# patrick-bedkowski/Generative-DNN-for-Physics-Simulations-CERN

Hardware: AMD Instinct MI355X
Metric: GAN-step images/sec (44x44 ZDC) at 1/2/4/8 MI355X; conv MFMA util % (higher is better)
Workload: dtype fp32

## Files before the change

### generative-dnn-for-physics-simulations-cern_amd/csrc/conv_common.h

```cpp
#pragma once
#include "common.h"

enum { MODE_FWD = 0, MODE_DGRAD = 1, MODE_WGRAD = 2 };

struct FastDiv {
  uint32_t m;
  int l;
};
static inline FastDiv mkdiv(uint32_t d) {
  FastDiv f;
  f.l = 0;
  while ((1ull << f.l) < d) ++f.l;
  f.m = (uint32_t)(((1ull << 32) * ((1ull << f.l) - d)) / d + 1);
  return f;
}
__device__ __forceinline__ int fdiv(int x, FastDiv f) {
  return (int)((__umulhi((uint32_t)x, f.m) + (uint32_t)x) >> f.l);
}

struct SubPixel {
  int on;
  int ph[4], pw[4];
  int p0[4], q0[4];
  int oh[4], ow[4];
// ... 56 lines not shown
}

__device__ __forceinline__ void conv_live_gemm(ConvArgs& a, int mode) {
  a.mslot = a.M;
  if (a.d.rows == nullptr) return;
  const int nl = conv_live(a), npx = conv_live_px(a);
  if (mode == MODE_WGRAD) a.Kd = min(nl * (a.Kd / a.d.N), npx);
  else a.M = min(nl * (a.M / a.d.N), npx);
}


struct DetRequest {
  float* ws;
  int64_t floats;
  int splits;
};
extern thread_local DetRequest g_det_req;

struct BnRedRequest {
  const void* x;
  const es_norm_t* nm;
  const es_chain_t* ch;
  float* part;
  int64_t floats;
  int chunks;
};
extern thread_local BnRedRequest g_bnr_req;



struct StatsRequest {
  float* part;
  int64_t floats;
  int chunks;
};
extern thread_local StatsRequest g_stats_req;

struct AffineRequest {
  const float* scale;
  const float* shift;
  int act;
  float slope;
  int fused;
};
extern thread_local AffineRequest g_aff_req;
int es_f32_split_level();

extern thread_local int g_ring_hit;

extern "C" int64_t es_weight_planes_offset(int64_t n);

int es_conv_ring_launch(ConvArgs& a, int mode, hipStream_t st);
int es_conv_ring_launch_f32(ConvArgs& a, int mode, hipStream_t st);
int64_t es_wgrad_f32_ring_floats(const es_conv_desc_t& d, const int64_t ys[4], const int64_t xs[4]);
int es_wgrad_f32_ring(const es_conv_desc_t& d, const void* dy, const int64_t ys[4], const void* x,
                      const int64_t xs[4], float* dw, float beta, float* ws, int64_t ws_floats, hipStream_t st);
int es_wgrad_ws_launch(int bn, bool sp, dim3 grid, const ConvArgs& a, float* wsc, int ngt, hipStream_t st);
void es_wgrad_reduce_plain(const float* ws, int splits, int K, int C, int R, int S, float* dw, float beta,
                           hipStream_t st);
```

### generative-dnn-for-physics-simulations-cern_amd/csrc/conv_mfma.hip

```cpp
#include <algorithm>
#include <cstdio>
#include <cstdlib>
#include <type_traits>

#include "conv_common.h"
#include "ring_common.h"
#include "split_fp32.h"


namespace {

constexpr int RT = 512;
constexpr int NSLOT = 3;
constexpr int SPB_PFD = 2;
constexpr int SPB_DMA_HI = 6;

bool g_ring_off = false;
int g_wgrad_ws = 1;

template <typename F>
struct lambda_arg : lambda_arg<decltype(&F::operator())> {};
template <typename C, typename R, typename A0, typename... As>
struct lambda_arg<R (C::*)(A0, As...) const> {
  typedef A0 type;
};


struct ClsReg {
  uint64_t v;
  __device__ __forceinline__ void init(const int* src) {
    uint32_t lo = ((uint32_t)(uint16_t)src[0]) | ((uint32_t)(uint16_t)src[1] << 16);
    uint32_t hi = ((uint32_t)(uint16_t)src[2]) | ((uint32_t)(uint16_t)src[3] << 16);
    v = ((uint64_t)(uint32_t)uni((int)hi) << 32) | (uint32_t)uni((int)lo);
  }
  __device__ __forceinline__ int operator()(int c) const { return (int)(short)(uint16_t)(v >> (16 * c)); }
};

template <int BK = 64>
__device__ __forceinline__ int swz_x(int row) {
  return BK == 64 ? ((row >> 1) & 7) : ((0x78 >> (2 * ((row >> 2) & 3))) & 3);
}
template <int BK = 64>
__device__ __forceinline__ int swz(int row, int chunk) { return row * (BK * 2) + ((chunk ^ swz_x<BK>(row)) << 4); }

typedef short short4_t __attribute__((ext_vector_type(4)));
typedef short short8_t __attribute__((ext_vector_type(8)));

template <int BROWS>
__device__ __forceinline__ int swz_tr(int k) {
  if constexpr (BROWS >= 128) return ((k & 3) << 1) | (((k >> 3) & 1) << 3);
  else return (((k >> 1) & 1) << 1) | (((k >> 3) & 1) << 2);
}

template <int BROWS>
__device__ __forceinline__ int tr_off(int k, int row) {
  return k * (BROWS * 2) + ((((row >> 3) ^ swz_tr<BROWS>(k)) << 4) | ((row & 7) << 1));
}

template <int BROWS>
__device__ __forceinline__ bf16x8 tr_frag(const char* img, int k0, int r0) {
  const int lane = threadIdx.x & 63;
  const int g = lane >> 4, q = (lane >> 2) & 3, p = lane & 3;
  const int ka = k0 + 8 * g + q;
  const char* p0 = img + tr_off<BROWS>(ka, r0 + 4 * p);
  const char* p1 = img + tr_off<BROWS>(ka + 4, r0 + 4 * p);
  short4_t lo = __builtin_amdgcn_ds_read_tr16_b64_v4i16((__attribute__((address_space(3))) short4_t*)p0);
  short4_t hi = __builtin_amdgcn_ds_read_tr16_b64_v4i16((__attribute__((address_space(3))) short4_t*)p1);
  short8_t v = {lo[0], lo[1], lo[2], lo[3], hi[0], hi[1], hi[2], hi[3]};
  return __builtin_bit_cast(bf16x8, v);
}

typedef int int2v __attribute__((ext_vector_type(2)));
typedef int int4v __attribute__((ext_vector_type(4)));
typedef unsigned int v4u32_t __attribute__((ext_vector_type(4)));
__device__ __forceinline__ uint32_t lds_u32(const void* p) {
  return (uint32_t)(uintptr_t)(const __attribute__((address_space(3))) void*)p;
}
__device__ __forceinline__ int2v ds_tr16(uint32_t addr) {
  int2v r;
  asm volatile("ds_read_b64_tr_b16 %0, %1" : "=v"(r) : "v"(addr));
  return r;
}
template <int BROWS>
__device__ __forceinline__ bf16x8 tr_frag_asm(uint32_t img, int k0, int r0) {
  const int lane = threadIdx.x & 63;
  const int g = lane >> 4, q = (lane >> 2) & 3, p = lane & 3;
  const int ka = k0 + 8 * g + q;
  const int2v lo = ds_tr16(img + tr_off<BROWS>(ka, r0 + 4 * p));
  const int2v hi = ds_tr16(img + tr_off<BROWS>(ka + 4, r0 + 4 * p));
  const int4v v = {lo[0], lo[1], hi[0], hi[1]};
  return __builtin_bit_cast(bf16x8, v);
}
__device__ __forceinline__ void fence_frag(bf16x8& x) {
  int4v v = __builtin_bit_cast(int4v, x);
  asm volatile("" : "+v"(v));
  x = __builtin_bit_cast(bf16x8, v);
// ... 2264 lines not shown
        for (int z = q; z < splits; z += WR_LANES, p += WR_LANES * zst) {
#pragma unroll
          for (int cl = 0; cl < 4; ++cl) {
            const float4 w = *(const float4*)(p + off[cl]);
            v.x += w.x; v.y += w.y; v.z += w.z; v.w += w.w;
          }
        }
      } else {
        const int off = (r * S + s) * C;
#pragma unroll 4
        for (int z = q; z < splits; z += WR_LANES, p += WR_LANES * zst) {
          const float4 w = *(const float4*)(p + off);
          v.x += w.x; v.y += w.y; v.z += w.z; v.w += w.w;
        }
      }
    }
    part[q][o] = v;
    __syncthreads();
    if (q == 0 && i < n4) {
      float4 u = part[0][o];
#pragma unroll
      for (int l = 1; l < WR_LANES; ++l) {
        const float4 w = part[l][o];
        u.x += w.x; u.y += w.y; u.z += w.z; u.w += w.w;
      }
      const float uu[4] = {u.x, u.y, u.z, u.w};
#pragma unroll
      for (int j = 0; j < 4; ++j) {
        float* g = dw + (((int64_t)k * C + c + j) * R + r) * S + s;
        *g = (beta != 0.f ? beta * *g : 0.f) + uu[j];
      }
    }
    __syncthreads();
  }
}

static void launch_wgrad_reduce(const float* ws, int splits, int K, int C, int R, int S, int ngt, const SubPixel& sp,
                                float* dw, float beta, hipStream_t st) {
  if (C % 4 == 0 && ngt % 4 == 0) {
    const int64_t n4 = (int64_t)K * C / 4 * R * S;
    const int blocks = (int)std::min<int64_t>((n4 + 31) / 32, 16384);
    hipLaunchKernelGGL(wgrad_reduce4_kernel, dim3(blocks), dim3(256), 0, st, ws, splits, K, C, R, S, ngt, sp, dw, beta);
    return;
  }
  const int64_t n = (int64_t)K * C * R * S;
  const int blocks = (int)std::min<int64_t>((n + 31) / 32, 16384);
  hipLaunchKernelGGL(wgrad_reduce_kernel, dim3(blocks), dim3(256), 0, st, ws, splits, K, C, R, S, ngt, sp, dw, beta);
}
int64_t g_conv_launches = 0;
extern "C" int64_t es_conv_launch_count() { return g_conv_launches; }

template <int MODE, int BM, int BN, bool SP, int BK, typename T, int SPL>
void launch_ring_grid(const ConvArgs& a, dim3 grid, hipStream_t st, bool aff) {
  if constexpr (MODE == MODE_FWD && (sizeof(T) == 2 || SPL > 0)) {
    if (aff) {
      g_aff_req.fused = 1;
      hipLaunchKernelGGL((conv_ring_kernel<MODE, BM, BN, SP, BK, T, SPL, true>), grid, dim3(RT), 0, st, a);
      return;
    }
  }
  hipLaunchKernelGGL((conv_ring_kernel<MODE, BM, BN, SP, BK, T, SPL>), grid, dim3(RT), 0, st, a);
}

template <int MODE, int BM, int BN, bool SP, int BK = 64, typename T = bf16, int SPL = 0>
void launch_ring(const ConvArgs& a, int row_tiles, hipStream_t st, bool aff = false) {
  dim3 grid(row_tiles, (a.Ng + BN - 1) / BN, 1);
  ++g_conv_launches;
  launch_ring_grid<MODE, BM, BN, SP, BK, T, SPL>(a, grid, st, aff);
}

constexpr int WGRAD_MINK = 8;
template <int BM, int BN, bool SP>
void launch_wgrad_ring(ConvArgs& a, hipStream_t st) {
  const int taps = SP ? a.sp.tap0[4] : a.d.R * a.d.S;
  const int tiles = (a.M / BM) * (taps * a.d.C / BN);
  int npix = a.d.P * a.d.Q;
  if (SP)
    for (int c = 0; c < 4; ++c) npix = c == 0 ? a.sp.ph[0] * a.sp.pw[0] : max(npix, a.sp.ph[c] * a.sp.pw[c]);
  const int ks = npix * ((a.d.N + 63) / 64);
  const int want = max(1, min(ks / WGRAD_MINK, 512 / tiles));
  const int per = (ks + want - 1) / want;
  a.k_per_split = per;
  dim3 grid(a.M / BM, taps * a.d.C / BN, (ks + per - 1) / per);
  ++g_conv_launches;
  hipLaunchKernelGGL((wgrad_ring_kernel<BM, BN, SP>), grid, dim3(RT), 0, st, a);
}

template <int EB>
bool dense_small_t(const int64_t s[4], int n, int c, int h, int w) {
  return s[1] == 1 && s[3] == c && s[2] == (int64_t)w * c && s[0] == (int64_t)h * w * c &&
         (int64_t)n * s[0] * EB < (1ll << 30);
}
bool dense_small(const int64_t s[4], int n, int c, int h, int w) { return dense_small_t<2>(s, n, c, h, w); }

constexpr int RING_NG = 64;
constexpr int RING_NG_DYN = 16;
bool g_subpixel_off = false;
bool g_ring256 = true;
bool g_persist = true;
bool g_p256 = true;

}

thread_local StatsRequest g_stats_req;
thread_local AffineRequest g_aff_req;
thread_local BnRedRequest g_bnr_req;

void es_make_subpixel(const es_conv_desc_t& d, int row_tile, SubPixel& sp) {
  int dhv[2], dwv[2], p0v[2], q0v[2], phv[2], pwv[2], ohv[2], owv[2];
  for (int a = 0; a < 2; ++a) {
    dhv[a] = ((a + d.R - 1) >> 1) + 1;
    dwv[a] = ((a + d.S - 1) >> 1) + 1;
    p0v[a] = (a + d.pad) & 1;
    q0v[a] = (a + d.pad) & 1;
    phv[a] = d.P > p0v[a] ? (d.P - p0v[a] + 1) / 2 : 0;
    pwv[a] = d.Q > q0v[a] ? (d.Q - q0v[a] + 1) / 2 : 0;
    ohv[a] = (p0v[a] - d.pad - a) / 2;
    owv[a] = (q0v[a] - d.pad - a) / 2;
  }
  sp.on = 1;
  sp.tap0[0] = 0;
  sp.tile0[0] = 0;
  for (int c = 0; c < 4; ++c) {
    const int a = c >> 1, b = c & 1;
    sp.ph[c] = phv[a];
    sp.pw[c] = pwv[b];
    sp.p0[c] = p0v[a];
    sp.q0[c] = q0v[b];
    sp.oh[c] = ohv[a];
    sp.ow[c] = owv[b];
    sp.dh[c] = dhv[a];
    sp.dw[c] = dwv[b];
    sp.tap0[c + 1] = sp.tap0[c] + dhv[a] * dwv[b];
    const int pix = phv[a] * pwv[b];
    sp.tile0[c + 1] = sp.tile0[c] + (row_tile > 0 ? (pix + row_tile - 1) / row_tile : 0);
  }
}

extern "C" int es_conv_set_ring(int on) {
  const int old = !g_ring_off;
  g_ring_off = !on;
  return old;
}

extern "C" int es_conv_set_persist(int on) {
  const int old = g_persist ? 1 : 0;
  g_persist = (on & 1) != 0;
  return old;
}

extern "C" int es_conv_set_p256(int on) {
  const int old = g_p256;
  g_p256 = on != 0;
  return old;
}

extern "C" int es_conv_set_ring256(int on) {
  const int old = g_ring256;
  g_ring256 = on != 0;
  return old;
}

extern "C" int es_conv_set_subpixel(int on) {
  const int old = !g_subpixel_off;
  g_subpixel_off = !on;
  return old;
}

extern "C" int es_subpixel_taps(int R, int S) {
  return (((R - 1) >> 1) + 1 + (R >> 1) + 1) * (((S - 1) >> 1) + 1 + (S >> 1) + 1);
}

extern "C" int es_conv_subpixel_ok(const es_conv_desc_t* d, es_dtype_t dt) {
  if (g_ring_off || g_subpixel_off || !d || (dt != ES_BF16 && dt != ES_F32)) return 0;
  if (d->up_h != 2 || d->up_w != 2 || d->hmap || d->stride != 1) return 0;
  if (d->C % 64 || d->K % 64) return 0;
  const int eb = dt == ES_F32 ? 4 : 2;
  const int64_t xbytes = (int64_t)d->N * d->H * d->W * d->C * eb, ybytes = (int64_t)d->N * d->P * d->Q * d->K * eb;
  const int64_t wbytes = (int64_t)d->K * d->C * es_subpixel_taps(d->R, d->S) * eb;
  if (dt == ES_F32) return wbytes < (1ll << 30) && (int64_t)d->H * d->W * d->C * eb < (1ll << 24) &&
                           (int64_t)d->P * d->Q * d->K * eb < (1ll << 24);
  (void)xbytes; (void)ybytes;
  return wbytes < (1ll << 30) && (int64_t)d->H * d->W * d->C * eb < (1ll << 24) &&
         (int64_t)d->P * d->Q * d->K * eb < (1ll << 24);
}

template <typename T, int SPL = 0>
int ring_fd(ConvArgs& a, int mode, hipStream_t st);
namespace {
int chunk_images(int64_t img_bytes, int N);
int ring_launch_chunks(ConvArgs& a, int mode, int nc, hipStream_t st);
}

int es_conv_ring_launch(ConvArgs& a, int mode, hipStream_t st) {
  const es_conv_desc_t& d = a.d;
  const bool sp_weights = d.subpixel != 0;
// ... 460 lines not shown
```

### generative-dnn-for-physics-simulations-cern_amd/csrc/ring_common.h

```cpp
#pragma once
#include "common.h"

namespace {

constexpr uint32_t OOB = 0x80000000u;

typedef __attribute__((address_space(3))) void lds_void;

__device__ __forceinline__ __amdgpu_buffer_rsrc_t mkres(const void* p, uint32_t bytes) {
  return __builtin_amdgcn_make_buffer_rsrc((void*)p, (short)0, (int)bytes, 0x00020000);
}
__device__ __forceinline__ void bdma16(__amdgpu_buffer_rsrc_t r, uint32_t voff, char* lds_wave_base) {
  __builtin_amdgcn_raw_ptr_buffer_load_lds(r, (lds_void*)lds_wave_base, 16, (int)voff, 0, 0, 0);
}

__device__ __forceinline__ void ring_barrier() { asm volatile("s_barrier" ::: "memory"); }

template <int N>
__device__ __forceinline__ void wait_vmcnt() {
  asm volatile("s_waitcnt vmcnt(%0)" ::"n"(N) : "memory");
}

__device__ __forceinline__ int xcd_remap(int orig, int nwg) {
  const int q8 = nwg / 8, r8 = nwg % 8, xcd = orig % 8;
  return (xcd < r8 ? xcd * (q8 + 1) : r8 * (q8 + 1) + (xcd - r8) * q8) + orig / 8;
}

__device__ __forceinline__ int uni(int v) { return __builtin_amdgcn_readfirstlane(v); }

}
```

### generative-dnn-for-physics-simulations-cern_amd/expertsim/hip.py

```python
from __future__ import annotations

import ctypes as C
import os

import numpy as np
import torch

_LIB_PATH = os.environ.get("ES_LIB") or os.path.join(os.path.dirname(os.path.abspath(__file__)), "_lib",
                                                     "libexpertsim_hip.so")
_lib = None

ES_F32, ES_BF16 = 0, 1
ACT_NONE, ACT_RELU, ACT_LRELU = 0, 1, 2
NORM_NONE, NORM_BN, NORM_GN, NORM_LN = 0, 1, 2, 3


class View(C.Structure):
    _fields_ = [("n", C.c_int), ("c", C.c_int), ("h", C.c_int), ("w", C.c_int), ("s", C.c_int64 * 4),
                ("rows", C.c_void_p)]


class Dropout(C.Structure):
    _fields_ = [("seed", C.c_uint64), ("stream", C.c_uint32), ("threshold", C.c_uint32),
                ("scale", C.c_float), ("enabled", C.c_int), ("step_ptr", C.c_void_p), ("step_mul", C.c_int32),
# ... 27 lines not shown
class DFront2Params(C.Structure):
    _fields_ = [("w1", C.c_void_p), ("sigma1", C.c_void_p), ("b1", C.c_void_p), ("g1", C.c_void_p),
                ("be1", C.c_void_p), ("w2", C.c_void_p), ("sigma2", C.c_void_p), ("b2", C.c_void_p),
                ("g2", C.c_void_p), ("be2", C.c_void_p), ("eps1", C.c_float), ("eps2", C.c_float),
                ("slope", C.c_float), ("ph", C.c_int), ("pw", C.c_int), ("rows", C.c_void_p)]


class DMlpParams(C.Structure):
    _fields_ = [("w1", C.c_void_p), ("sigma1", C.c_void_p), ("b1", C.c_void_p), ("g1", C.c_void_p),
                ("be1", C.c_void_p), ("w2", C.c_void_p), ("sigma2", C.c_void_p), ("b2", C.c_void_p),
                ("g2", C.c_void_p), ("be2", C.c_void_p), ("w3", C.c_void_p), ("sigma3", C.c_void_p),
                ("b3", C.c_void_p), ("eps1", C.c_float), ("eps2", C.c_float), ("slope", C.c_float),
                ("rows", C.c_void_p)]


class PackJob(C.Structure):
    _fields_ = [("w", C.c_void_p), ("K", C.c_int), ("C", C.c_int), ("R", C.c_int), ("S", C.c_int),
                ("mode", C.c_int), ("dt", C.c_int), ("planes", C.c_int), ("out", C.c_void_p)]


class Affine(C.Structure):
    _fields_ = [("scale", C.c_void_p), ("shift", C.c_void_p), ("act", C.c_int), ("slope", C.c_float)]


P = C.c_void_p
I64 = C.c_int64
_SIGS = {
    "es_last_error": (C.c_char_p, []),
    "es_version": (C.c_int, []),
    "es_device_sync": (C.c_int, []),
    "es_conv_set_glds": (C.c_int, [C.c_int]),
    "es_conv_set_ring": (C.c_int, [C.c_int]),
    "es_conv_set_subpixel": (C.c_int, [C.c_int]),
    "es_conv_set_ring256": (C.c_int, [C.c_int]),
    "es_conv_set_persist": (C.c_int, [C.c_int]),
    "es_conv_set_p256": (C.c_int, [C.c_int]),
    "es_conv_subpixel_ok": (C.c_int, [P, C.c_int]),
    "es_subpixel_taps": (C.c_int, [C.c_int, C.c_int]),
    "es_conv2d_fwd": (C.c_int, [P, C.c_int, P, P, P, P, P, C.c_int, P, P]),
    "es_conv2d_fwd_stats": (C.c_int, [P, C.c_int, P, P, P, P, P, C.c_int, P, P, I64, P, P]),
    "es_conv2d_fwd_affine": (C.c_int, [P, C.c_int, P, P, P, P, P, P, C.c_int, P, P, P]),
    "es_conv2d_dgrad": (C.c_int, [P, C.c_int, P, P, P, P, C.c_int, P, C.c_float, P]),
    "es_conv2d_dgrad_bnred": (C.c_int, [P, C.c_int, P, P, P, P, C.c_int, P, P, P, P, P, I64, P, P]),
    "es_conv2d_wgrad": (C.c_int, [P, C.c_int, P, P, P, P, P, P]),
    "es_conv2d_wgrad_det_ws_bytes": (I64, [P, C.c_int, P, P]),
    "es_conv2d_wgrad_det": (C.c_int, [P, C.c_int, P, P, P, P, P, C.c_float, P, I64, P]),
    "es_set_deterministic": (C.c_int, [C.c_int]),
    "es_conv2d_splitk_ws_bytes": (I64, [P, C.c_int]),
    "es_conv2d_fwd_det": (C.c_int, [P, C.c_int, P, P, P, P, P, C.c_int, P, P, I64, P]),
    "es_conv2d_dgrad_det": (C.c_int, [P, C.c_int, P, P, P, P, C.c_int, P, P, I64, P]),
    "es_conv_set_f32_chunk": (C.c_int, [C.c_int]),
    "es_conv_set_f32_split": (C.c_int, [C.c_int]),
    "es_conv_set_wgrad_ws": (C.c_int, [C.c_int]),
    "es_weight_planes_offset": (C.c_int64, [C.c_int64]),
    "es_pack_weight_planes": (C.c_int, [P, C.c_int64, P, P]),
    "es_pack_conv_weights": (C.c_int, [P, C.c_int, P]),
    "es_conv_launch_count": (C.c_int64, []),
    "es_conv_exec_flops": (C.c_int, [C.POINTER(C.c_double), C.c_int]),
    "es_pack_conv_weight": (C.c_int, [P, C.c_int, C.c_int, C.c_int, C.c_int, C.c_int, P, P, P, C.c_int, P]),
    "es_unpack_conv_grad": (C.c_int, [P, C.c_int, C.c_int, C.c_int, C.c_int, P, P, C.c_float, P]),
    "es_unpack_conv_grad_clear": (C.c_int, [P, C.c_int, C.c_int, C.c_int, C.c_int, P, C.c_float, P]),
    "es_norm_stats_ws_bytes": (I64, [P, C.c_int, C.c_int]),
    "es_norm_stats": (C.c_int, [P, C.c_int, P, C.c_int, C.c_int, C.c_float, P, P, P, P, C.c_float, P, P]),
    "es_norm_act_fwd": (C.c_int, [P, C.c_int, P, P, P, C.c_int, P, P, P, C.c_int, P, P]),
    "es_norm_stats_finalize": (C.c_int, [P, C.c_int, C.c_int, C.c_float, P, P, P, P, C.c_float, P]),
    "es_norm_bwd_ws_bytes": (I64, [P, C.c_int, C.c_int]),
    "es_norm_act_bwd": (C.c_int, [P, C.c_int, P, P, P, P, C.c_int, P, P, C.c_int, P, P, C.c_int, P,
                                  C.c_float, P, P, P, P, P]),
    "es_norm_act_bwd_sums": (C.c_int, [P, C.c_int, P, P, P, P, C.c_int, P, P, C.c_int, P, P, C.c_int, P, P, P,
                                       P, P]),
    "es_norm_stats_merge": (C.c_int, [P, C.c_int, C.c_int, P, P]),
    "es_norm_stats_local": (C.c_int, [P, C.c_int, P, P, P, P]),
    "es_norm_bwd_sync": (C.c_int, [C.c_int, P, C.c_int, P, P, P, P, C.c_int, P, P, C.c_int, P, P, C.c_float, P, P,
                                   P, P, P, P]),
    "es_act_fwd": (C.c_int, [P, C.c_int, P, P, P, C.c_int, P, P]),
    "es_dropout_keep_bits": (C.c_int, [P, P, P]),
    "es_channel_sum_ws_bytes": (I64, [P]),
    "es_channel_sum": (C.c_int, [P, C.c_int, P, P, C.c_float, P, P]),
    "es_maxpool_fwd": (C.c_int, [P, C.c_int, P, C.c_int, C.c_int, C.c_int, C.c_int, P, P, P, P]),
    "es_maxpool_bwd": (C.c_int, [P, C.c_int, P, P, C.c_int, C.c_int, C.c_int, C.c_int, P, P, C.c_float, P]),
    "es_dfront_fwd": (C.c_int, [P, P, C.c_int, C.c_int, C.c_int, P, P, P, P, P, C.c_float, C.c_float, P, P, P, P,
                                P]),
    "es_dfront_part_floats": (I64, [C.c_int]),
    "es_dfront_bwd": (C.c_int, [P, P, C.c_int, C.c_int, C.c_int, P, P, P, P, P, C.c_float, C.c_float, P, P, P, P,
                                P, P, P, P, P, P, P, P]),
    "es_dfront2_ok": (C.c_int, [C.c_int, C.c_int, C.c_int, C.c_int]),
    "es_dfront2_part_floats": (I64, [C.c_int]),
    "es_dfront2_save_floats": (I64, [C.c_int, C.c_int, C.c_int, C.c_int]),
    "es_dfront2_fwd": (C.c_int, [P, P, C.c_int, C.c_int, C.c_int, P, P, P, I64, P, P]),
    "es_dfront2_bwd": (C.c_int, [P, P, C.c_int, C.c_int, C.c_int, P, P, P, P, I64, P, P, P, P, P, P, P, P, P, P,
                                 P, P]),
    "es_dfront2_set_probe": (None, [P]),
    "es_dmlp_part_floats": (I64, [C.c_int, C.c_int]),
    "es_dmlp_fwd": (C.c_int, [P, I64, C.c_int, C.c_int, P, P, P, P, P, P, P, P]),
    "es_dmlp_bwd": (C.c_int, [P, I64, C.c_int, C.c_int, P, P, P, P, P, P, P, P, P, I64, P, P, P, P, P, P, P, P, P,
                              P, P, P]),
    "es_upsample_bwd": (C.c_int, [P, C.c_int, P, P, P, P, P, P, C.c_int, P, C.c_float, P]),
    "es_upsample_fwd": (C.c_int, [P, C.c_int, P, P, P, P, P, P]),
    "es_copy": (C.c_int, [P, C.c_int, P, P, C.c_int, P, C.c_float, C.c_float, P]),
    "es_avgpool_fwd": (C.c_int, [P, C.c_int, P, P, P, P]),
    "es_avgpool_bwd": (C.c_int, [P, P, P, C.c_int, P, C.c_float, P]),
    "es_gather_rows": (C.c_int, [P, I64, P, C.c_int, C.c_int, P, I64, P]),
    "es_gather_rows_at": (C.c_int, [P, I64, P, P, C.c_int, C.c_int, P, I64, P, P]),
    "es_scatter_rows_at": (C.c_int, [P, P, P, C.c_int, P, P, P]),
    "es_sn_power_iter": (C.c_int, [P, C.c_int, C.c_int, P, P, P, C.c_int, P, P]),
    "es_sn_power_iter_batch": (C.c_int, [C.c_int, P, P, P, P, P, P, C.c_int, P, P]),
# ... 227 lines not shown
```

### include/expertsim_hip.h

```cpp
#ifndef EXPERTSIM_HIP_H
#define EXPERTSIM_HIP_H

#include <stdint.h>

#ifdef __cplusplus
extern "C" {
#endif

typedef enum { ES_F32 = 0, ES_BF16 = 1 } es_dtype_t;
enum { ES_OK = 0, ES_ERR_ARG = 1, ES_ERR_HIP = 2, ES_ERR_UNSUPPORTED = 3 };
enum { ES_ACT_NONE = 0, ES_ACT_RELU = 1, ES_ACT_LRELU = 2 };
enum { ES_NORM_NONE = 0, ES_NORM_BN = 1, ES_NORM_GN = 2, ES_NORM_LN = 3 };

typedef void* es_stream_t;

typedef struct {
  int n, c, h, w;
  int64_t s[4];
  const int32_t* rows;
} es_view_t;

typedef struct {
  uint64_t seed;
  uint32_t stream;
// ... 17 lines not shown
  int K, P, Q;
  int R, S;
  int stride, pad;
  const int32_t* hmap;
  const int32_t* wmap;
  int up_h, up_w;
  int subpixel;
  const int32_t* rows;
  int rows_px;
} es_conv_desc_t;

int es_conv_set_glds(int on);
int es_conv_set_ring(int on);
int es_conv_set_ring256(int on);
int es_conv_set_persist(int on);
int es_conv_set_p256(int on);
int es_conv_set_subpixel(int on);
int es_conv_subpixel_ok(const es_conv_desc_t* d, es_dtype_t dt);
int es_subpixel_taps(int R, int S);

int es_conv2d_fwd(const es_conv_desc_t* d, es_dtype_t dt, const void* x, const int64_t xs[4],
                  const void* wk, const float* bias, void* y, es_dtype_t ydt, const int64_t ys[4],
                  es_stream_t stream);
int es_conv2d_fwd_stats(const es_conv_desc_t* d, es_dtype_t dt, const void* x, const int64_t xs[4],
                        const void* wk, const float* bias, void* y, es_dtype_t ydt, const int64_t ys[4],
                        float* part, int64_t part_floats, int* chunks, es_stream_t stream);
typedef struct {
  const float* scale;
  const float* shift;
  int act;
  float slope;
} es_affine_t;
int es_conv2d_fwd_affine(const es_conv_desc_t* d, es_dtype_t dt, const void* x, const int64_t xs[4],
                         const void* wk, const float* bias, const es_affine_t* epi, void* y, es_dtype_t ydt,
                         const int64_t ys[4], int* fused, es_stream_t stream);
int es_conv2d_dgrad(const es_conv_desc_t* d, es_dtype_t dt, const void* dy, const int64_t ys[4],
                    const void* wd, void* dxu, es_dtype_t dxdt, const int64_t dxs[4], float beta,
                    es_stream_t stream);
int es_conv2d_wgrad(const es_conv_desc_t* d, es_dtype_t dt, const void* dy, const int64_t ys[4],
                    const void* x, const int64_t xs[4], float* dw, es_stream_t stream);
int64_t es_conv2d_wgrad_det_ws_bytes(const es_conv_desc_t* d, es_dtype_t dt, const int64_t ys[4],
                                     const int64_t xs[4]);
int es_conv2d_wgrad_det(const es_conv_desc_t* d, es_dtype_t dt, const void* dy, const int64_t ys[4],
                        const void* x, const int64_t xs[4], float* dw, float beta, void* ws, int64_t ws_bytes,
                        es_stream_t stream);
int64_t es_conv2d_splitk_ws_bytes(const es_conv_desc_t* d, int mode);
int es_conv2d_fwd_det(const es_conv_desc_t* d, es_dtype_t dt, const void* x, const int64_t xs[4], const void* wk,
                      const float* bias, void* y, es_dtype_t ydt, const int64_t ys[4], void* ws, int64_t ws_bytes,
                      es_stream_t stream);
int es_conv2d_dgrad_det(const es_conv_desc_t* d, es_dtype_t dt, const void* dy, const int64_t ys[4], const void* wd,
                        void* dxu, es_dtype_t dxdt, const int64_t dxs[4], void* ws, int64_t ws_bytes,
                        es_stream_t stream);
int es_conv_set_wgrad_ws(int on);
int es_set_deterministic(int on);
int es_conv_set_f32_chunk(int images);
int es_conv_set_f32_split(int on);
int64_t es_weight_planes_offset(int64_t n);
int es_pack_weight_planes(const float* packed, int64_t n, void* base, es_stream_t stream);
int64_t es_conv_launch_count(void);
int es_conv_exec_flops(double out[3], int reset);

int es_pack_conv_weight(const float* w, int K, int C, int R, int S, int mode,
                        const float* inv_scale, const int32_t* col_perm, void* out, es_dtype_t dt,
                        es_stream_t stream);
typedef struct {
  const float* w;
  int K, C, R, S, mode;
  int dt;
  int planes;
  void* out;
} es_pack_job_t;
int es_pack_conv_weights(const es_pack_job_t* jobs, int n, es_stream_t stream);
int es_unpack_conv_grad(const float* dw, int K, int C, int R, int S, const int32_t* col_perm,
                        float* grad, float beta, es_stream_t stream);
int es_unpack_conv_grad_clear(float* dw, int K, int C, int R, int S, float* grad, float beta,
                              es_stream_t stream);

typedef struct {
  int kind;
  int groups;
  const float* mean;
  const float* invstd;
  const float* gamma;
  const float* beta;
} es_norm_t;

typedef struct {
  es_dropout_t drop;
  int dropout_first;
  int act;
  float slope;
  uint8_t* keep;
  int keep_ready;
} es_chain_t;

int64_t es_norm_stats_ws_bytes(const es_view_t* x, int kind, int groups);
int es_norm_stats(const es_view_t* x, es_dtype_t xdt, const void* xp, int kind, int groups,
                  float eps, float* mean, float* invstd, float* running_mean, float* running_var,
                  float momentum, void* ws, es_stream_t stream);
int es_norm_stats_finalize(const float* part, int chunks, int C, float eps, float* mean, float* invstd,
                           float* running_mean, float* running_var, float momentum, es_stream_t stream);
int es_norm_act_fwd(const es_view_t* x, es_dtype_t xdt, const es_norm_t* nm, const es_chain_t* ch,
                    const es_view_t* addend, es_dtype_t adt, const void* addend_ptr, const void* xp,
                    const es_view_t* y, es_dtype_t ydt, void* yp, es_stream_t stream);
int64_t es_norm_bwd_ws_bytes(const es_view_t* x, int kind, int groups);
int es_norm_act_bwd(const es_view_t* x, es_dtype_t xdt, const void* xp, const es_norm_t* nm,
// ... 187 lines not shown
```

Measured before the change: 24180.

## Add persistent split-fp32 ring conv kernel with cross-tile prefetch

```diff
diff --git a/generative-dnn-for-physics-simulations-cern_amd/csrc/conv_common.h b/generative-dnn-for-physics-simulations-cern_amd/csrc/conv_common.h
--- a/generative-dnn-for-physics-simulations-cern_amd/csrc/conv_common.h
+++ b/generative-dnn-for-physics-simulations-cern_amd/csrc/conv_common.h
@@ -132,6 +132,8 @@
 
 int es_conv_ring_launch(ConvArgs& a, int mode, hipStream_t st);
 int es_conv_ring_launch_f32(ConvArgs& a, int mode, hipStream_t st);
+int es_ring_persist32_launch(int mode, int bm, int bn, bool sp, bool aff, bool all, const ConvArgs& a, dim3 grid,
+                             hipStream_t st);
 int64_t es_wgrad_f32_ring_floats(const es_conv_desc_t& d, const int64_t ys[4], const int64_t xs[4]);
 int es_wgrad_f32_ring(const es_conv_desc_t& d, const void* dy, const int64_t ys[4], const void* x,
                       const int64_t xs[4], float* dw, float beta, float* ws, int64_t ws_floats, hipStream_t st);
diff --git a/generative-dnn-for-physics-simulations-cern_amd/csrc/conv_mfma.hip b/generative-dnn-for-physics-simulations-cern_amd/csrc/conv_mfma.hip
--- a/generative-dnn-for-physics-simulations-cern_amd/csrc/conv_mfma.hip
+++ b/generative-dnn-for-physics-simulations-cern_amd/csrc/conv_mfma.hip
@@ -12,11 +12,11 @@
 
 constexpr int RT = 512;
 constexpr int NSLOT = 3;
-constexpr int SPB_PFD = 2;
-constexpr int SPB_DMA_HI = 6;
 
 bool g_ring_off = false;
 int g_wgrad_ws = 1;
+int g_ring_persist32 = 1;
+int64_t g_ring_persist32_launches = 0;
 
 template <typename F>
 struct lambda_arg : lambda_arg<decltype(&F::operator())> {};
@@ -26,22 +26,6 @@
 };
 
 
-struct ClsReg {
-  uint64_t v;
-  __device__ __forceinline__ void init(const int* src) {
-    uint32_t lo = ((uint32_t)(uint16_t)src[0]) | ((uint32_t)(uint16_t)src[1] << 16);
-    uint32_t hi = ((uint32_t)(uint16_t)src[2]) | ((uint32_t)(uint16_t)src[3] << 16);
-    v = ((uint64_t)(uint32_t)uni((int)hi) << 32) | (uint32_t)uni((int)lo);
-  }
-  __device__ __forceinline__ int operator()(int c) const { return (int)(short)(uint16_t)(v >> (16 * c)); }
-};
-
-template <int BK = 64>
-__device__ __forceinline__ int swz_x(int row) {
-  return BK == 64 ? ((row >> 1) & 7) : ((0x78 >> (2 * ((row >> 2) & 3))) & 3);
-}
-template <int BK = 64>
-__device__ __forceinline__ int swz(int row, int chunk) { return row * (BK * 2) + ((chunk ^ swz_x<BK>(row)) << 4); }
 
 typedef short short4_t __attribute__((ext_vector_type(4)));
 typedef short short8_t __attribute__((ext_vector_type(8)));
@@ -2412,6 +2396,14 @@
 
 template <int MODE, int BM, int BN, bool SP, int BK, typename T, int SPL>
 void launch_ring_grid(const ConvArgs& a, dim3 grid, hipStream_t st, bool aff) {
+  if constexpr (SPL == 2 && BK == 64) {
+    if (g_ring_persist32 &&
+        es_ring_persist32_launch(MODE, BM, BN, SP, aff, g_ring_persist32 == 2, a, grid, st) == 1) {
+      if (aff) g_aff_req.fused = 1;
+      ++g_ring_persist32_launches;
+      return;
+    }
+  }
   if constexpr (MODE == MODE_FWD && (sizeof(T) == 2 || SPL > 0)) {
     if (aff) {
       g_aff_req.fused = 1;
@@ -2502,6 +2494,14 @@
   g_ring_off = !on;
   return old;
 }
+
+extern "C" int es_conv_set_ring_persist32(int on) {
+  const int old = g_ring_persist32;
+  g_ring_persist32 = on < 0 ? 0 : (on > 2 ? 2 : on);
+  return old;
+}
+
+extern "C" int64_t es_conv_ring_persist32_count(void) { return g_ring_persist32_launches; }
 
 extern "C" int es_conv_set_persist(int on) {
   const int old = g_persist ? 1 : 0;
diff --git a/generative-dnn-for-physics-simulations-cern_amd/csrc/conv_ring_persist32.hip b/generative-dnn-for-physics-simulations-cern_amd/csrc/conv_ring_persist32.hip
--- /dev/null
+++ b/generative-dnn-for-physics-simulations-cern_amd/csrc/conv_ring_persist32.hip
@@ -0,0 +1,620 @@
+#include <algorithm>
+#include <type_traits>
+
+#include "conv_common.h"
+#include "ring_common.h"
+#include "split_fp32.h"
+
+namespace {
+
+constexpr int RT = 512;
+
+typedef int int4p __attribute__((ext_vector_type(4)));
+__device__ __forceinline__ uint32_t lds_addr(const void* p) {
+  return (uint32_t)(uintptr_t)(const __attribute__((address_space(3))) void*)p;
+}
+__device__ __forceinline__ void lds_write_b32(uint32_t addr, float v) {
+  asm volatile("ds_write_b32 %0, %1" ::"v"(addr), "v"(v) : "memory");
+}
+__device__ __forceinline__ void lds_write_b16(uint32_t addr, uint32_t v) {
+  asm volatile("ds_write_b16 %0, %1" ::"v"(addr), "v"(v) : "memory");
+}
+__device__ __forceinline__ int4p lds_read_b128(uint32_t addr) {
+  int4p r;
+  asm volatile("ds_read_b128 %0, %1" : "=v"(r) : "v"(addr) : "memory");
+  return r;
+}
+__device__ __forceinline__ void wait_lgkm0() { asm volatile("s_waitcnt lgkmcnt(0)" ::: "memory"); }
+
+template <int MODE, int BM, int BN, bool SP, bool AFF>
+__global__ void __launch_bounds__(RT) conv_ring_persist32_kernel(ConvArgs a, int gx, int nt) {
+  static_assert(!AFF || MODE == MODE_FWD, "affine epilogue: FWD only");
+  static_assert((BM == 256 && (BN == 64 || BN == 128)) || (BM == 128 && BN == 128), "SPB tiles with a 3-slot A ring");
+  constexpr int BK = 64, NW = 8, NT = 64 * NW;
+  constexpr int WGM = NW, WM = BM / WGM, WN = BN;
+  constexpr int RM = WM / 16, RN = WN / 16;
+  constexpr int ROWB = BK * 2, PROWS = 1024 / ROWB;
+  constexpr int EB = 4, BKC = ROWB / EB, EA = EB, CPR = ROWB / 16, EBB = 6;
+  constexpr int BPL = BN / 16, BPIECES = 3 * BPL;
+  constexpr int APW = BM / PROWS / NW, BPW = (BPIECES + NW - 1) / NW;
+  constexpr int ABYTES = BM * ROWB, BBYTES = 3 * BN * 64;
+  constexpr bool SPLITD = 3 * (ABYTES + BBYTES) > 144 * 1024;
+  constexpr int NSA = 3, NSB = SPLITD ? 2 : 3;
+  constexpr int LOOPWAIT = (NSA - 2) * APW + (NSB - 2) * BPW;
+  constexpr int BOFF = 2 * ABYTES, A2OFF = BOFF + NSB * BBYTES, RINGB = A2OFF + ABYTES;
+  constexpr int STB = 3 * WGM * BN * 4;
+  constexpr int JUNK = BPW * NW > BPIECES ? 1024 : 0;
+  constexpr int LDS_MAX = 160 * 1024;
+  constexpr int FREE0 = BOFF + BBYTES, FREEB = RINGB - FREE0;
+  constexpr int PITCH = WN * 4 + 16;
+  constexpr int SR = (WM >= 16 && NW * 16 * PITCH <= FREEB + (LDS_MAX - RINGB - STB - JUNK)) ? 16 : 8;
+  constexpr int STAGE = NW * SR * PITCH;
+  constexpr int EXTRA = STAGE > FREEB ? STAGE - FREEB : 0;
+  constexpr int TOTAL = RINGB + EXTRA + STB + JUNK;
+  static_assert(TOTAL <= LDS_MAX && WM % SR == 0, "LDS plan");
+  __shared__ __attribute__((aligned(16))) char smem[TOTAL];
+  char* const junk = smem + RINGB + EXTRA + STB;
+  const es_conv_desc_t& d = a.d;
+  const int NL = conv_live(a);
+  const SubPixel& sp = a.sp;
+
+  const int NG = a.ng, PPG = NG / PROWS;
+  const int NB = BM / NG;
+  int TT;
+  if constexpr (MODE == MODE_FWD && SP) TT = a.sp_merge ? sp.tile0[1] : (a.sp_tpc > 0 ? 4 * a.sp_tpc : sp.tile0[4]);
+  else if constexpr (MODE == MODE_FWD) TT = (d.P * d.Q + NB - 1) / NB;
+  else TT = ((a.fold ? d.H * d.W : d.Hu * d.Wu) + NB - 1) / NB;
+  const int ntot = gx * nt;
+  const int nlive = NL == d.N ? ntot : min(ntot, (NL + NG - 1) / NG * TT * nt);
+  int s_beg, s_end, s_step;
+  {
+    const int bid = blockIdx.x, xcd = bid & 7, lw = bid >> 3, L = ((int)gridDim.x - xcd + 7) >> 3;
+    const int q8 = nlive / 8, r8 = nlive % 8;
+    const int x_lo = xcd < r8 ? xcd * (q8 + 1) : r8 * (q8 + 1) + (xcd - r8) * q8, x_cnt = q8 + (xcd < r8 ? 1 : 0);
+    s_beg = x_lo + lw;
+    s_end = x_lo + x_cnt;
+    s_step = L;
+  }
+
+  const int lane = threadIdx.x & 63, wid = uni(threadIdx.x >> 6);
+  const int wm0 = wid * WM;
+  const int lrow = lane / CPR, pc = lane % CPR;
+
+  const __amdgpu_buffer_rsrc_t ares = mkres(a.a_src, (uint32_t)(NL * a.as[0] * EA));
+  int bbytes;
+  if constexpr (SP && MODE == MODE_FWD) bbytes = sp.tap0[4] * a.Ng * d.C * EBB;
+  else if constexpr (SP) bbytes = a.Ng * sp.tap0[4] * d.K * EBB;
+  else bbytes = a.Ng * ((MODE == MODE_DGRAD && a.fold) ? d.R * d.S * d.K : a.Kd) * EBB;
+  const __amdgpu_buffer_rsrc_t bres = mkres(a.b_src, (uint32_t)bbytes);
+  const int as2b = (int)a.as[2] * EA, as3b = (int)a.as[3] * EA;
+  const int nch = MODE == MODE_FWD ? d.C : d.K;
+  const int upw = d.up_w > 0 ? d.up_w : 1;
+  ClsReg Roh, Row, Rph, Rpw, Rp0, Rq0, Rtap0, Rdh, Rdw;
+  if constexpr (SP && MODE == MODE_DGRAD) {
+    Roh.init(sp.oh); Row.init(sp.ow); Rph.init(sp.ph); Rpw.init(sp.pw); Rp0.init(sp.p0); Rq0.init(sp.q0);
+    Rtap0.init(sp.tap0); Rdh.init(sp.dh); Rdw.init(sp.dw);
+  }
+
+  struct Hdr {
+    int tl, n0, cls, gw, PQ, gi, pix0;
+  };
+  Hdr nx{0, 0, 0, 1, 0, 0, 0}, cu{0, 0, 0, 1, 0, 0, 0};
+  auto decode_hdr = [&](int s) -> bool {
+    const int tl = s / nt, n0 = (s - tl * nt) * BN;
+    int cls = 0, gh, gw, jt;
+    if constexpr (MODE == MODE_FWD && SP) {
+      if (a.sp_merge) {
+        jt = tl % TT;
+      } else if (a.sp_tpc > 0) {
+        const int r = tl % TT;
+        cls = r & 3;
+        jt = r >> 2;
+        if (jt >= sp.tile0[cls + 1] - sp.tile0[cls]) {
+          if (a.stats_part) {
+            float* pp = a.stats_part + (int64_t)tl * 3 * a.Ng;
+            for (int c = threadIdx.x; c < BN; c += NT)
+              if (n0 + c < a.Ng) pp[n0 + c] = 0.f;
+          }
+          return false;
+        }
+      } else {
+        const int r = tl % TT;
+        cls = (r >= sp.tile0[1]) + (r >= sp.tile0[2]) + (r >= sp.tile0[3]);
+        jt = r - sp.tile0[cls];
+      }
+      gh = sp.ph[cls];
+      gw = sp.pw[cls];
+    } else {
+      if constexpr (MODE == MODE_FWD) {
+        gh = d.P;
+        gw = d.Q;
+      } else {
+        gh = a.fold ? d.H : d.Hu;
+        gw = a.fold ? d.W : d.Wu;
+      }
+      jt = tl % TT;
+    }
+    const int gi = tl / TT;
+    if (gi * NG >= NL) {
+      if (MODE == MODE_FWD && a.stats_part) {
+        for (int c = threadIdx.x; c < BN; c += NT) {
+          const int gc = n0 + c, cc = a.sp_merge ? gc / a.Ng : 0, ch = gc - cc * a.Ng;
+          if (cc < 4 && ch < a.Ng) {
+            float* pp = a.stats_part + (int64_t)(a.sp_merge ? tl * 4 + cc : tl) * 3 * a.Ng;
+            pp[ch] = 0.f;
+            pp[a.Ng + ch] = 0.f;
+            pp[2 * a.Ng + ch] = 0.f;
+          }
+        }
+      }
+      return false;
+    }
+    nx = Hdr{tl, n0, cls, gw, gh * gw, gi, jt * NB};
+    return true;
+  };
+  for (int s = nlive + (int)blockIdx.x; s < ntot; s += (int)gridDim.x) decode_hdr(s);
+
+  uint32_t alane[APW];
+  int pc0[APW], pc1[APW];
+  bool pval[APW];
+  uint32_t blane[BPW];
+  int ldb = 0, nk = 0, bper = 1;
+  int cr = 0, cs = 0, cch = 0, cua = 0, cub = 0, ckb = 0, ccls = 0, cstep = 0;
+  int kh = 1, kw = 1;
+  uint32_t ua_t[APW];
+  int bs = 0, bsm = 0;
+  auto decode_addr = [&]() {
+    const int cls = nx.cls, gw = nx.gw;
+    int bbase = 0;
+    if constexpr (SP && MODE == MODE_FWD) {
+      ldb = sp.dh[cls] * sp.dw[cls] * d.C;
+      bbase = sp.tap0[cls] * a.Ng * d.C;
+    } else if constexpr (SP) {
+      ldb = sp.tap0[4] * d.K;
+    } else {
+      ldb = (MODE == MODE_DGRAD && a.fold) ? d.R * d.S * d.K : a.Kd;
+    }
+#pragma unroll
+    for (int j = 0; j < APW; ++j) {
+      const int pi = wid * APW + j;
+      const int rr = pi * PROWS + lrow;
+      const int lc = pc ^ swz_x<BK>(rr);
+      const int ppix = pi / PPG;
+      const int pix = nx.pix0 + ppix;
+      pval[j] = pix < nx.PQ;
+      const int pp = pval[j] ? pix : 0;
+      const int y = pp / gw, x = pp - y * gw;
+      const int img = nx.gi * NG + (pi - ppix * PPG) * PROWS + lrow;
+      alane[j] = (uint32_t)(img * (int)a.as[0] * EB + lc * 16);
+      if constexpr (MODE == MODE_FWD && SP) {
+        pc0[j] = y + sp.oh[cls];
+        pc1[j] = x + sp.ow[cls];
+      } else if constexpr (MODE == MODE_FWD) {
+        pc0[j] = y * d.stride - d.pad;
+        pc1[j] = x * d.stride - d.pad;
+      } else if constexpr (SP) {
+        pc0[j] = y;
+        pc1[j] = x;
+      } else if (a.fold) {
+        pc0[j] = y * d.up_h + d.pad;
+        pc1[j] = x * d.up_w + d.pad;
+      } else {
+        pc0[j] = y + d.pad;
+        pc1[j] = x + d.pad;
+      }
+      ua_t[j] = OOB;
+    }
+#pragma unroll
+    for (int j = 0; j < BPW; ++j) {
+      const int q = wid * BPW + j;
+      const int rr = (q % BPL) * 16 + (lane >> 2);
+      blane[j] = q < BPIECES ? (uint32_t)((bbase + (nx.n0 + rr) * ldb) * EBB + (q / BPL) * 64 +
+                                          (((lane & 3) ^ swz_x<32>(rr)) * 16))
+                             : OOB;
+    }
+    if constexpr (SP) nk = ldb / BKC;
+    else nk = a.Kd / BKC;
+    bper = (MODE == MODE_DGRAD && !SP) ? (d.R * d.S * d.K) / BKC : nk;
+    cr = cs = cch = cua = cub = ckb = ccls = cstep = 0;
+    bs = bsm = 0;
+    kh = SP ? uni(sp.dh[cls]) : d.R;
+    kw = SP ? uni(sp.dw[cls]) : d.S;
+  };
+  auto issue = [&](char* slot) {
+    if (cch == 0) {
+      const bool live = cstep < nk;
+#pragma unroll
+      for (int j = 0; j < APW; ++j) {
+        uint32_t u;
+        if constexpr (MODE == MODE_FWD && SP) {
+          const int hs = pc0[j] + cr, ws = pc1[j] + cs;
+          const bool ok = live && pval[j] && (unsigned)hs < (unsigned)d.H && (unsigned)ws < (unsigned)d.W;
+          u = ok ? (uint32_t)(hs * as2b + ws * as3b) : OOB;
+        } else if constexpr (MODE == MODE_FWD) {
+          const int hu = pc0[j] + cr, wu = pc1[j] + cs;
+          const bool ok = live && pval[j] && (unsigned)hu < (unsigned)d.Hu && (unsigned)wu < (unsigned)d.Wu;
+          const int sh = fdiv(hu, a.fUh), sw = fdiv(wu, a.fUw);
+          u = ok ? (uint32_t)(sh * as2b + sw * as3b) : OOB;
+        } else if constexpr (SP) {
+          const int uu = pc0[j] - cr - Roh(ccls), vv = pc1[j] - cs - Row(ccls);
+          const bool ok = live && pval[j] && (unsigned)uu < (unsigned)Rph(ccls) &&
+                          (unsigned)vv < (unsigned)Rpw(ccls);
+          u = ok ? (uint32_t)((Rp0(ccls) + 2 * uu) * as2b + (Rq0(ccls) + 2 * vv) * as3b) : OOB;
+        } else {
+          const int ph = pc0[j] + cua - cr, pw = pc1[j] + cub - cs;
+          const int sh = d.stride == 2 ? 1 : 0;
+          const bool ok = live && pval[j] && ph >= 0 && pw >= 0 && !(((ph | pw) & sh)) &&
+                          (ph >> sh) < d.P && (pw >> sh) < d.Q;
+          u = ok ? (uint32_t)((ph >> sh) * as2b + (pw >> sh) * as3b) : OOB;
+        }
+        ua_t[j] = u;
+      }
+    }
+    const uint32_t co = (uint32_t)(cch * EA);
+#pragma unroll
+    for (int j = 0; j < APW; ++j) bdma16(ares, alane[j] + (ua_t[j] + co), slot + (wid * APW + j) * 1024);
+    ++cstep;
+    cch += BKC;
+    if (cch == nch) {
+      cch = 0;
+      ckb += nch;
+      ++cs;
+      const bool w2 = cs == kw;
+      cs = w2 ? 0 : cs;
+      cr += w2;
+      const bool w3 = cr == kh;
+      cr = w3 ? 0 : cr;
+      ckb = w3 ? 0 : ckb;
+      cub += w3;
+      const bool w4 = cub == upw;
+      cub = w4 ? 0 : cub;
+      cua += w4;
+      if constexpr (SP && MODE == MODE_DGRAD) {
+        ccls += w3;
+        const int cn = ccls < 4 ? ccls : 3;
+        kh = Rdh(cn);
+        kw = Rdw(cn);
+      }
+    }
+  };
+  auto issue_b = [&](char* bslot) {
+    const uint32_t ub = bs < nk ? (uint32_t)(bsm * BKC * EBB) : OOB;
+#pragma unroll
+    for (int j = 0; j < BPW; ++j) {
+      const int q = wid * BPW + j;
+      char* dst = (!JUNK || q < BPIECES) ? bslot + q * 1024 : junk;
+      bdma16(bres, blane[j] + ub, dst);
+    }
+    ++bs;
+    bsm = bsm + 1 == bper ? 0 : bsm + 1;
+  };
+  auto aslot = [&](int i) -> char* { return smem + (i == 2 ? A2OFF : i * ABYTES); };
+  char* const bring = smem + BOFF;
+
+  const int r16 = lane & 15, g16 = lane >> 4;
+  auto rd_a = [&](f32x4 (&r)[RM][2], const char* as) {
+#pragma unroll
+    for (int i = 0; i < RM; ++i)
+#pragma unroll
+      for (int h = 0; h < 2; ++h) r[i][h] = *(const f32x4*)(as + swz<BK>(wm0 + i * 16 + r16, g16 + 4 * h));
+  };
+  auto rd_b = [&](bf16x8 (&bp)[3], const char* bimg, int j) {
+#pragma unroll
+    for (int pl = 0; pl < 3; ++pl)
+      bp[pl] = *(const bf16x8*)(bimg + pl * (BN * 64) + swz<32>(j * 16 + r16, g16));
+  };
+
+  const int lgNG = uni(31 - __builtin_clz(NG));
+  const int NLP = conv_live_px(a);
+  FastDiv fgw{0, 0};
+  int fgw_of = 0;
+  float (*st_n)[BN] = (float (*)[BN])(smem + RINGB + EXTRA);
+  float (*st_m)[BN] = st_n + WGM;
+  float (*st_q)[BN] = st_n + 2 * WGM;
+  const uint32_t stg = lds_addr(smem + FREE0 + wid * (SR * PITCH));
+
+  if (a.prio && wid >= 4) __builtin_amdgcn_s_setprio(1);
+
+  int seq = s_beg;
+  auto advance = [&]() -> bool {
+    while (seq < s_end) {
+      if (decode_hdr(seq)) {
+        decode_addr();
+        return true;
+      }
+      seq += s_step;
+    }
+    return false;
+  };
+  auto prefetch = [&]() {
+    issue(aslot(0));
+    issue_b(bring);
+    issue(aslot(1));
+  };
+  bool have = advance();
+  if (have) prefetch();
+  while (have) {
+    cu = nx;
+    f32x4 acc[RM][RN];
+#pragma unroll
+    for (int i = 0; i < RM; ++i)
+#pragma unroll
+      for (int j = 0; j < RN; ++j) acc[i][j] = f32x4{0.f, 0.f, 0.f, 0.f};
+    wait_vmcnt<0>();
+    ring_barrier();
+    if constexpr (NSB == 3) issue_b(bring + BBYTES);
+    issue(aslot(2));
+    const int nkc = nk;
+    bf16x8 apc[RM][3];
+    {
+      f32x4 r[RM][2];
+      rd_a(r, aslot(0));
+#pragma unroll
+      for (int i = 0; i < RM; ++i) split8(r[i][0], r[i][1], apc[i]);
+    }
+    int sa1 = 1, sb = 0, ia = 0, ib = NSB - 1;
+    constexpr int JS = RN > 2 ? RN / 2 : RN - 1;
+    constexpr int JDMA = SPB_DMA_HI < RN ? SPB_DMA_HI : RN - 1;
+    for (int t = 0; t < nkc; ++t) {
+      wait_vmcnt<LOOPWAIT>();
+      asm volatile("s_waitcnt lgkmcnt(0)" ::: "memory");
+      ring_barrier();
+      const char* bimg = bring + sb * BBYTES;
+      constexpr int PFD = SPB_PFD;
+      bf16x8 bq[PFD + 1][3];
+#pragma unroll
+      for (int j = 0; j < PFD && j < RN; ++j) rd_b(bq[j], bimg, j);
+      f32x4 ra[RM][2];
+      rd_a(ra, aslot(sa1));
+      bf16x8 apn[RM][3];
+#pragma unroll
+      for (int j = 0; j < RN; ++j) {
+        if (j + PFD < RN) rd_b(bq[(j + PFD) % (PFD + 1)], bimg, j + PFD);
+#pragma unroll
+        for (int i = 0; i < RM; ++i) acc[i][j] = mfma_split6(apc[i], bq[j % (PFD + 1)], acc[i][j]);
+        if (j == (wid >= 4 ? JDMA : 0)) {
+          issue_b(bring + ib * BBYTES);
+          issue(aslot(ia));
+        }
+        if (j == JS) {
+#pragma unroll
+          for (int i = 0; i < RM; ++i) split8(ra[i][0], ra[i][1], apn[i]);
+        }
+      }
+#pragma unroll
+      for (int i = 0; i < RM; ++i)
+#pragma unroll
+        for (int pl = 0; pl < 3; ++pl) apc[i][pl] = apn[i][pl];
+      sa1 = sa1 + 1 == NSA ? 0 : sa1 + 1;
+      ia = ia + 1 == NSA ? 0 : ia + 1;
+      sb = sb + 1 == NSB ? 0 : sb + 1;
+      ib = ib + 1 == NSB ? 0 : ib + 1;
+    }
+    wait_vmcnt<0>();
+
+    int el = lane;
+    asm volatile("" : "+v"(el));
+    const int col16 = el & 15, rq = (el >> 4) * 4;
+    const int gw = cu.gw, PQ = cu.PQ, gi = cu.gi, pix0 = cu.pix0, tl = cu.tl;
+    if (gw != fgw_of) {
+      uint32_t l = 0;
+      while ((1u << l) < (uint32_t)gw) ++l;
+      fgw.l = uni((int)l);
+      fgw.m = (uint32_t)uni((int)(uint32_t)(((1ull << 32) * ((1ull << l) - (uint32_t)gw)) / (uint32_t)gw + 1));
+      fgw_of = gw;
+    }
+    auto row_pix = [&](int r) { return pix0 + ((wm0 + r) >> lgNG); };
+    auto row_img = [&](int r) { return gi * NG + ((wm0 + r) & (NG - 1)); };
+    int ecls = cu.cls, kc0 = cu.n0;
+    if constexpr (SP && MODE == MODE_FWD) {
+      if (a.sp_merge) {
+        ecls = kc0 / a.Ng;
+        kc0 -= ecls * a.Ng;
+      }
+    }
+    auto row_off = [&](int r) -> int64_t {
+      const int pix = row_pix(r);
+      int y = fdiv(pix, fgw), x = pix - y * gw;
+      if constexpr (SP && MODE == MODE_FWD) {
+        y = sp.p0[ecls] + 2 * y;
+        x = sp.q0[ecls] + 2 * x;
+      }
+      return (int64_t)row_img(r) * a.os[0] + (int64_t)y * a.os[2] + (int64_t)x * a.os[3];
+    };
+    auto row_ok = [&](int r) { return row_pix(r) < PQ && row_img(r) < NL && row_img(r) * PQ + row_pix(r) < NLP; };
+#pragma unroll
+    for (int j = 0; j < RN; ++j) {
+      const int ng = kc0 + j * 16 + col16;
+      float bv = 0.f;
+      if constexpr (MODE == MODE_FWD) bv = (a.bias && ng < a.Ng) ? a.bias[ng] : 0.f;
+      if constexpr (AFF) {
+        const float sc = ng < a.Ng ? a.epi_scale[ng] : 0.f;
+        const float sh = fmaf(bv, sc, ng < a.Ng ? a.epi_shift[ng] : 0.f);
+        const float neg = a.epi_act == ES_ACT_LRELU ? a.epi_slope : (a.epi_act == ES_ACT_RELU ? 0.f : 1.f);
+#pragma unroll
+        for (int i = 0; i < RM; ++i)
+#pragma unroll
+          for (int jj = 0; jj < 4; ++jj) {
+            float v = fmaf(acc[i][j][jj], sc, sh);
+            v = v > 0.f ? v : v * neg;
+            acc[i][j][jj] = a.out_bf16 ? (float)(bf16)v : v;
+          }
+      } else {
+#pragma unroll
+        for (int i = 0; i < RM; ++i)
+#pragma unroll
+          for (int jj = 0; jj < 4; ++jj) {
+            const float v = acc[i][j][jj] + bv;
+            acc[i][j][jj] = a.out_bf16 ? (float)(bf16)v : v;
+          }
+      }
+    }
+    float* part = MODE == MODE_FWD ? a.stats_part : nullptr;
+    if (part) {
+      bool okr[RM][4];
+#pragma unroll
+      for (int i = 0; i < RM; ++i)
+#pragma unroll
+        for (int jj = 0; jj < 4; ++jj) okr[i][jj] = row_ok(i * 16 + rq + jj);
+#pragma unroll
+      for (int j = 0; j < RN; ++j) {
+        float n_, m_, q;
+        float cnt = 0.f, s = 0.f;
+#pragma unroll
+        for (int i = 0; i < RM; ++i)
+#pragma unroll
+          for (int jj = 0; jj < 4; ++jj)
+            if (okr[i][jj]) { cnt += 1.f; s += acc[i][j][jj]; }
+        const float mu = cnt > 0.f ? s / cnt : 0.f;
+        q = 0.f;
+#pragma unroll
+        for (int i = 0; i < RM; ++i)
+#pragma unroll
+          for (int jj = 0; jj < 4; ++jj)
+            if (okr[i][jj]) { const float e = acc[i][j][jj] - mu; q += e * e; }
+        n_ = cnt; m_ = mu;
+#pragma unroll
+        for (int o = 16; o <= 32; o <<= 1) {
+          const float nb = __shfl_xor(n_, o, 64), mb = __shfl_xor(m_, o, 64), qb = __shfl_xor(q, o, 64);
+          const float nt2 = n_ + nb;
+          if (nt2 > 0.f) {
+            const float dl = mb - m_, f = nb / nt2;
+            m_ += dl * f;
+            q += qb + dl * dl * n_ * f;
+          }
+          n_ = nt2;
+        }
+        if (el < 16) {
+          st_n[wid][j * 16 + col16] = n_;
+          st_m[wid][j * 16 + col16] = m_;
+          st_q[wid][j * 16 + col16] = q;
+        }
+      }
+    }
+    __syncthreads();
+
+    seq += s_step;
+    have = advance();
+    if (have) prefetch();
+
+    auto stage_store = [&](auto ec) {
+      constexpr int ESZ = decltype(ec)::value;
+      constexpr int PITCHE = WN * ESZ + 16;
+      constexpr int CPRO = WN * ESZ / 16;
+      constexpr int RPI = 64 / CPRO;
+      constexpr int NIT = SR / RPI;
+      static_assert(NIT >= 1 && SR % RPI == 0, "staging pass");
+      const int lr = el / CPRO, lch = el % CPRO;
+      const bool colok = kc0 + lch * 16 / ESZ < a.Ng;
+      char* obase = (char*)a.out + (int64_t)kc0 * ESZ + lch * 16;
+#pragma unroll
+      for (int ps = 0; ps < WM / SR; ++ps) {
+        constexpr int PPB = 16 / SR;
+        const int i = ps / PPB;
+        const bool mine = PPB == 1 || (el >> 5) == (ps % PPB);
+        const int rl = PPB == 1 ? rq : (rq & 4);
+        if (mine) {
+#pragma unroll
+          for (int jj = 0; jj < 4; ++jj)
+#pragma unroll
+            for (int j = 0; j < RN; ++j) {
+              const uint32_t p = stg + (rl + jj) * PITCHE + (j * 16 + col16) * ESZ;
+              const float v = acc[i][j][jj];
+              if constexpr (ESZ == 2) lds_write_b16(p, (uint32_t)__builtin_bit_cast(uint16_t, (bf16)v));
+              else lds_write_b32(p, v);
+            }
+        }
+        wait_lgkm0();
+        int4p vals[NIT];
+#pragma unroll
+        for (int it = 0; it < NIT; ++it) vals[it] = lds_read_b128(stg + (it * RPI + lr) * PITCHE + lch * 16);
+        wait_lgkm0();
+#pragma unroll
+        for (int it = 0; it < NIT; ++it) asm volatile("" : "+v"(vals[it]));
+        if (colok) {
+#pragma unroll
+          for (int it = 0; it < NIT; ++it) {
+            const int r = ps * SR + it * RPI + lr;
+            if (row_ok(r)) {
+              const int64_t ro = row_off(r);
+              *(uint4*)(obase + ro * ESZ) = __builtin_bit_cast(uint4, vals[it]);
+            }
+          }
+        }
+      }
+    };
+    if (a.out_bf16) stage_store(std::integral_constant<int, 2>{});
+    else stage_store(std::integral_constant<int, 4>{});
+
+    if (part && wid == 0) {
+      for (int c = el; c < WN; c += 64) {
+        float n_ = st_n[0][c], m_ = st_m[0][c], q = st_q[0][c];
+        for (int w = 1; w < WGM; ++w) {
+          const float nb = st_n[w][c];
+          if (nb > 0.f) {
+            const float mb = st_m[w][c], nt2 = n_ + nb, dl = mb - m_, f = nb / nt2;
+            m_ += dl * f;
+            q += st_q[w][c] + dl * dl * n_ * f;
+            n_ = nt2;
+          }
+        }
+        const int kc = kc0 + c;
+        if (kc < a.Ng) {
+          float* pp = part + (int64_t)(a.sp_merge ? tl * 4 + ecls : tl) * 3 * a.Ng;
+          pp[kc] = n_;
+          pp[a.Ng + kc] = m_;
+          pp[2 * a.Ng + kc] = q;
+        }
+      }
+    }
+  }
+  wait_vmcnt<0>();
+}
+
+int g_ncu = 0;
+
+template <int MODE, int BM, int BN, bool SP>
+void launch_p32(const ConvArgs& a, dim3 grid, bool aff, hipStream_t st) {
+  const int ntot = (int)(grid.x * grid.y);
+  const int nwg = std::min(ntot, g_ncu);
+  if constexpr (MODE == MODE_FWD) {
+    if (aff) {
+      hipLaunchKernelGGL((conv_ring_persist32_kernel<MODE, BM, BN, SP, true>), dim3(nwg), dim3(RT), 0, st, a,
+                         (int)grid.x, (int)grid.y);
+      return;
+    }
+  }
+  hipLaunchKernelGGL((conv_ring_persist32_kernel<MODE, BM, BN, SP, false>), dim3(nwg), dim3(RT), 0, st, a,
+                     (int)grid.x, (int)grid.y);
+}
+
+}
+
+int es_ring_persist32_launch(int mode, int bm, int bn, bool sp, bool aff, bool all, const ConvArgs& a, dim3 grid,
+                             hipStream_t st) {
+  if (!a.vec_out || grid.z != 1) return 0;
+  if (g_ncu == 0) {
+    int dev = 0, n = 0;
+    if (hipGetDevice(&dev) != hipSuccess || hipDeviceGetAttribute(&n, hipDeviceAttributeMultiprocessorCount, dev) != hipSuccess ||
+        n <= 0)
+      return 0;
+    g_ncu = n;
+  }
+#define ES_P32(MD, BMV, BNV, SPV, DFLT)                                         \
+  if (mode == MD && bm == BMV && bn == BNV && sp == SPV) {                      \
+    if (!(DFLT) && !all) return 0;                                              \
+    launch_p32<MD, BMV, BNV, SPV>(a, grid, aff, st);                            \
+    return 1;                                                                   \
+  }
+  ES_P32(MODE_FWD, 256, 64, false, false)
+  ES_P32(MODE_DGRAD, 256, 128, false, true)
+  ES_P32(MODE_FWD, 256, 128, true, false)
+  ES_P32(MODE_DGRAD, 256, 128, true, false)
+  ES_P32(MODE_DGRAD, 128, 128, true, false)
+  ES_P32(MODE_FWD, 256, 64, true, false)
+  ES_P32(MODE_FWD, 256, 128, false, false)
+  ES_P32(MODE_DGRAD, 256, 64, false, false)
+  ES_P32(MODE_DGRAD, 256, 64, true, false)
+#undef ES_P32
+  return 0;
+}
diff --git a/generative-dnn-for-physics-simulations-cern_amd/csrc/ring_common.h b/generative-dnn-for-physics-simulations-cern_amd/csrc/ring_common.h
--- a/generative-dnn-for-physics-simulations-cern_amd/csrc/ring_common.h
+++ b/generative-dnn-for-physics-simulations-cern_amd/csrc/ring_common.h
@@ -28,4 +28,24 @@
 
 __device__ __forceinline__ int uni(int v) { return __builtin_amdgcn_readfirstlane(v); }
 
+constexpr int SPB_PFD = 2;
+constexpr int SPB_DMA_HI = 6;
+
+struct ClsReg {
+  uint64_t v;
+  __device__ __forceinline__ void init(const int* src) {
+    uint32_t lo = ((uint32_t)(uint16_t)src[0]) | ((uint32_t)(uint16_t)src[1] << 16);
+    uint32_t hi = ((uint32_t)(uint16_t)src[2]) | ((uint32_t)(uint16_t)src[3] << 16);
+    v = ((uint64_t)(uint32_t)uni((int)hi) << 32) | (uint32_t)uni((int)lo);
+  }
+  __device__ __forceinline__ int operator()(int c) const { return (int)(short)(uint16_t)(v >> (16 * c)); }
+};
+
+template <int BK = 64>
+__device__ __forceinline__ int swz_x(int row) {
+  return BK == 64 ? ((row >> 1) & 7) : ((0x78 >> (2 * ((row >> 2) & 3))) & 3);
 }
+template <int BK = 64>
+__device__ __forceinline__ int swz(int row, int chunk) { return row * (BK * 2) + ((chunk ^ swz_x<BK>(row)) << 4); }
+
+}
diff --git a/generative-dnn-for-physics-simulations-cern_amd/expertsim/hip.py b/generative-dnn-for-physics-simulations-cern_amd/expertsim/hip.py
--- a/generative-dnn-for-physics-simulations-cern_amd/expertsim/hip.py
+++ b/generative-dnn-for-physics-simulations-cern_amd/expertsim/hip.py
@@ -103,6 +103,8 @@
     "es_conv_set_f32_chunk": (C.c_int, [C.c_int]),
     "es_conv_set_f32_split": (C.c_int, [C.c_int]),
     "es_conv_set_wgrad_ws": (C.c_int, [C.c_int]),
+    "es_conv_set_ring_persist32": (C.c_int, [C.c_int]),
+    "es_conv_ring_persist32_count": (C.c_int64, []),
     "es_weight_planes_offset": (C.c_int64, [C.c_int64]),
     "es_pack_weight_planes": (C.c_int, [P, C.c_int64, P, P]),
     "es_pack_conv_weights": (C.c_int, [P, C.c_int, P]),
diff --git a/include/expertsim_hip.h b/include/expertsim_hip.h
--- a/include/expertsim_hip.h
+++ b/include/expertsim_hip.h
@@ -93,6 +93,8 @@
                         void* dxu, es_dtype_t dxdt, const int64_t dxs[4], void* ws, int64_t ws_bytes,
                         es_stream_t stream);
 int es_conv_set_wgrad_ws(int on);
+int es_conv_set_ring_persist32(int on);
+int64_t es_conv_ring_persist32_count(void);
 int es_set_deterministic(int on);
 int es_conv_set_f32_chunk(int images);
 int es_conv_set_f32_split(int on);
```

After: 24120. About the same (-0.2%).
